# auggiemarignier/pxmcmc

Hardware: AMD Instinct MI355X
Metric: MYULA samples/sec at L=256 synthesis (higher is better)
Workload: dtype f64

## Files before the change

### pxmcmc_amd/csrc/sht_gemm.hip

```cpp
#include "../../include/pxmcmc_amd.h"
#include "sht_core.h"

#include <type_traits>

#include <hip/hip_ext.h>

#include <cstdlib>
#include <map>
#include <mutex>

namespace pxm {

typedef double d4 __attribute__((ext_vector_type(4)));

constexpr int KC = 16;
#define PXM_GEMM_MFMA(ACC, A, B) ACC = __builtin_amdgcn_mfma_f64_16x16x4f64(A, B, ACC, 0, 0, 0);
#ifdef PXM_GEMM_TRACE
__device__ unsigned long long* g_gemm_trace = nullptr;
extern "C" int pxm_debug_set_gemm_trace(unsigned long long* buf) {
  return hipMemcpyToSymbol(HIP_SYMBOL(g_gemm_trace), &buf, sizeof(buf)) == hipSuccess ? 0 : -1;
}
#endif
__device__ __forceinline__ double stage_add(double a, double b, bool on) { return a + (on ? b : 0.0); }
__device__ __forceinline__ double2 stage_add(double2 a, double2 b, bool on) { return double2{a.x + (on ? b.x : 0.0), a.y + (on ? b.y : 0.0)}; }
__device__ __forceinline__ double stage_scale(double a, double sc) { return a * sc; }
__device__ __forceinline__ double2 stage_scale(double2 a, double sc) { return double2{a.x * sc, a.y * sc}; }
template <int CT, int NSLAB>
struct GemmGeom {
  static constexpr int NCT = CT * NSLAB;
  static constexpr int COLS = 16 * NCT;
  static constexpr int PITCH = COLS + (COLS == 16 ? 0 : 16);
};
template <int CT, int NSLAB, int NW, int RT, int NSET, bool TWO, bool SK, int PK = 0, bool POLE = false>
__device__ __forceinline__ void sht_gemm_body(const GemmTask* __restrict__ tasks, const int bid,
                                              const double* __restrict__ X, double* __restrict__ Y, int ncol, int col0,
                                              const GemmAffine& aff, double (*xs)[KC][GemmGeom<CT, NSLAB>::PITCH]) {
  constexpr int NCT = CT * NSLAB;
  constexpr bool HOIST = TWO;
  constexpr int COLS = GemmGeom<CT, NSLAB>::COLS;
  constexpr int PITCH = GemmGeom<CT, NSLAB>::PITCH;
  constexpr int NT = 64 * NW;
  constexpr int VW = (KC * COLS / 2 >= NT) ? 2 : 1;
  constexpr int NV = KC * COLS / VW;
  constexpr int IT = (NV + NT - 1) / NT;
  const GemmTask t = tasks[bid];
  const int tid = threadIdx.x, lane = tid & 63;
  if (t.n_rt == 0) return;
  const int xn = (PK || TWO) ? t.x_ncol : ncol, yn = (PK || TWO) ? t.y_ncol : ncol;
#ifdef PXM_GEMM_TRACE
  const unsigned long long trace_t0 = wall_clock64();
  unsigned long long trace_t1 = 0, trace_t2 = 0;
  long long trace_c[5] = {0, 0, 0, 0, 0};
#define PXM_GEMM_CSTAMP(K) if (ch == 8) trace_c[K] = clock64();
#else
#define PXM_GEMM_CSTAMP(K)
#endif
  const int wave = __builtin_amdgcn_readfirstlane(tid >> 6);
  const int kq = lane >> 4, cl = lane & 15;
  const int n_my = min(RT, max(0, t.n_rt - RT * wave));
  const int nch = (t.k_end - t.k_beg) / KC;

  const double* sp[IT];
  const double* sp2[IT];
  const double* skp[IT];
  int so[IT];
  bool sv[IT];
#pragma unroll
  for (int i = 0; i < IT; ++i) {
    const int q0 = tid + NT * i;
    const int q = q0 % NV;
    const int kr = (q / (COLS / VW)) % KC, col = VW * (q % (COLS / VW));
    const int slab = PK ? ((col / (PK ? PK : 1)) < tasks[bid].nslab ? col / (PK ? PK : 1) : 0) : col / (16 * CT);
    const int cin = PK ? col % (PK ? PK : 1) : col % (16 * CT);
    sv[i] = q0 < NV;
    const int64_t xo = tasks[bid].x_off[slab];
    sp[i] = X + xo + col0 + cin + (int64_t)(t.k_beg + kr) * xn;
    sp2[i] = sp[i];
    skp[i] = sp[i];
    if (TWO) {
      const int64_t x2o = tasks[bid].x2_off[slab];
      if (x2o) sp2[i] = sp[i] + (x2o - xo);
    }
    if (SK) {
      const int64_t ks = tasks[bid].ks_off[slab >> 1];
      if (ks) skp[i] = X + ks + t.k_beg + kr;
    }
    so[i] = kr * PITCH + col;
  }
  const bool two = TWO && t.x2_off[0] != 0;
  const bool has_sk = SK && t.ks_off[0] != 0;
  typedef typename std::conditional<VW == 2, double2, double>::type stage_t;
  stage_t st[NSET - 1][IT], st2[NSET - 1][IT];
  double ssc[NSET - 1][IT];
#define PXM_STAGE_LOAD(SET, CH)                                                                     \
  {                                                                                                 \
    const int cs = min((CH), nch - 1);                                                              \
    _Pragma("unroll") for (int i = 0; i < IT; ++i) {                                                \
      st[SET][i] = *reinterpret_cast<const stage_t*>(sp[i] + (int64_t)cs * KC * xn);                \
      if (TWO) st2[SET][i] = *reinterpret_cast<const stage_t*>(sp2[i] + (int64_t)cs * KC * xn);   \
      if (SK) ssc[SET][i] = skp[i][cs * KC];                                                        \
    }                                                                                               \
  }
#define PXM_STAGE_STORE(SET, BUF)                                                                   \
  _Pragma("unroll") for (int i = 0; i < IT; ++i) {                                                  \
    stage_t v = st[SET][i];                                                                         \
    if (TWO) v = stage_add(v, st2[SET][i], two);                                                    \
    if (SK) {                                                                                       \
      v = stage_scale(v, has_sk ? ssc[SET][i] : 1.0);                                               \
    }                                                                                               \
    if (sv[i]) *reinterpret_cast<stage_t*>(&xs[BUF][0][0] + so[i]) = v;                             \
  }

  const double2* tab[RT];
#pragma unroll
  for (int r = 0; r < RT; ++r)
    tab[r] = reinterpret_cast<const double2*>(X + t.tab_off + (int64_t)(n_my > r ? RT * wave + r : 0) * t.rt_stride) + lane;
  const bool v0 = n_my > 0;
  double2 A[NSET][RT][2];
#define PXM_TAB_LOAD(SET, CH)                                                 \
  {                                                                           \
    const int cc = min((CH), nch - 1);                                        \
    _Pragma("unroll") for (int r = 0; r < RT; ++r) {                          \
      A[SET][r][0] = tab[r][(int64_t)(2 * cc) * 64];                          \
      A[SET][r][1] = tab[r][(int64_t)(2 * cc + 1) * 64];                      \
    }                                                                         \
  }

  d4 acc[RT][NCT];
#pragma unroll
  for (int r = 0; r < RT; ++r)
#pragma unroll
    for (int c = 0; c < NCT; ++c) acc[r][c] = d4{0, 0, 0, 0};

#pragma unroll
  for (int u = 0; u < NSET - 1; ++u)
#pragma unroll
    for (int i = 0; i < IT; ++i) {
      st[u][i] = st2[u][i] = stage_t{};
      ssc[u][i] = 0.0;
    }
  constexpr int PER = NSET * (NSET - 1);
  const int nit = nch + NSET - 1;
  for (int it0 = 0; it0 < nit; it0 += PER) {
#pragma unroll
    for (int pv = 0; pv < PER; ++pv) {
      const int it = it0 + pv;
      const int ch = it - (NSET - 1);
      constexpr int LAG = NSET - 1;
      const int us = pv % (NSET - 1);
      const int ut = pv % NSET;
      const int um = (pv + NSET - LAG % NSET) % NSET;
      const int buf = (pv + PER - LAG) & 1;
      PXM_GEMM_CSTAMP(0)
#ifdef PXM_GEMM_TRACE
      if (ch == 9) trace_c[4] = clock64();
#endif
      PXM_STAGE_STORE(us, buf)
      PXM_GEMM_CSTAMP(1)
      PXM_STAGE_LOAD(us, it)
      PXM_TAB_LOAD(ut, it)
      __syncthreads();
#ifdef PXM_GEMM_TRACE
      if (ch == 0) trace_t1 = wall_clock64();
#endif
      PXM_GEMM_CSTAMP(2)
      if (v0 && ch >= 0 && ch < nch) {
#define PXM_MFMA_CHUNK(NC)                                                                                     \
  {                                                                                                            \
    double b[4][NC];     \
    _Pragma("unroll") for (int h4 = 0; h4 < 4; ++h4)                                                           \
      _Pragma("unroll") for (int c = 0; c < NC; ++c) b[h4][c] = xs[buf][4 * h4 + kq][16 * c + cl];             \
    if (HOIST) __builtin_amdgcn_sched_barrier(0);  \
    _Pragma("unroll") for (int h4 = 0; h4 < 4; ++h4)                                                           \
      _Pragma("unroll") for (int r = 0; r < RT; ++r) {                                                         \
        const double av = (h4 & 1) ? A[um][r][h4 >> 1].y : A[um][r][h4 >> 1].x;                                \
        _Pragma("unroll") for (int c = 0; c < NC; ++c)                                                         \
            PXM_GEMM_MFMA(acc[r][c], av, b[h4][c])                                                             \
      }                                                                                                        \
  }
        PXM_MFMA_CHUNK(NCT)
#undef PXM_MFMA_CHUNK
      }
      PXM_GEMM_CSTAMP(3)
    }
  }
#undef PXM_STAGE_LOAD
#undef PXM_STAGE_STORE
#undef PXM_TAB_LOAD
#ifdef PXM_GEMM_TRACE
  trace_t2 = wall_clock64();
#endif

  constexpr int NGRP = PK ? 2 : 1;
  double hdv[RT][NSLAB][4], rsv[RT][NGRP][4];
#pragma unroll
  for (int r = 0; r < RT; ++r) {
    const int rowb = t.row0 + 16 * (r < n_my ? RT * wave + r : 0) + kq;
#pragma unroll
    for (int sl = 0; sl < NSLAB; ++sl)
#pragma unroll
      for (int q = 0; q < 4; ++q)
        hdv[r][sl][q] = (aff.on && t.hd_off[sl]) ? (X + t.hd_off[sl])[(int64_t)(rowb + 4 * q) * t.hd_stride + (cl & 1)] : 0.0;
#pragma unroll
    for (int g = 0; g < NGRP; ++g)
#pragma unroll
      for (int q = 0; q < 4; ++q) rsv[r][g][q] = t.rs_off[g] ? (X + t.rs_off[g])[rowb + 4 * q] : 1.0;
  }
  if constexpr (POLE) {
    if (t.pole_n) {
      constexpr int W2 = 8 * CT;
      constexpr int NRG = NT / W2;
      const int cp = tid % W2, rg = tid / W2;
      const double* xo = X + t.x_off[0] + t.pole_dx + col0 + 2 * cp;
      const double* xo2 = two ? X + t.x2_off[0] + t.pole_dx + col0 + 2 * cp : xo;
      const double* bo = X + t.pole_bo_off;
      double bown[RT][4];
#pragma unroll
      for (int r = 0; r < RT; ++r)
#pragma unroll
        for (int q = 0; q < 4; ++q)
          bown[r][q] = (X + t.pole_b_off)[t.row0 + 16 * (r < n_my ? RT * wave + r : 0) + kq + 4 * q];
      double2 part{0.0, 0.0};
#pragma unroll 1
      for (int r = rg; r < t.pole_n; r += NRG) {
        const double2 a = *reinterpret_cast<const double2*>(xo + (int64_t)r * xn);
        const double2 a2 = *reinterpret_cast<const double2*>(xo2 + (int64_t)r * xn);
        const double bv = bo[r];
        const double2 v = stage_add(a, a2, two);
        part.x += bv * v.x;
        part.y += bv * v.y;
      }
#pragma unroll
      for (int msk = W2; msk < 64; msk <<= 1) {
        part.x += __shfl_xor(part.x, msk);
        part.y += __shfl_xor(part.y, msk);
      }
      double* red = &xs[0][0][0];
      __syncthreads();
      if (lane < W2) *reinterpret_cast<double2*>(red + wave * 2 * W2 + 2 * lane) = part;
      __syncthreads();
#pragma unroll
      for (int ct = 0; ct < CT; ++ct) {
        double sc = 0.0;
#pragma unroll
        for (int w = 0; w < NW; ++w) sc += red[w * 2 * W2 + 16 * ct + cl];
#pragma unroll
        for (int r = 0; r < RT; ++r)
#pragma unroll
          for (int sl = 0; sl < NSLAB; ++sl)
#pragma unroll
            for (int q = 0; q < 4; ++q) acc[r][sl * CT + ct][q] += 0.5 * bown[r][q] * sc;
      }
    }
  }
  if constexpr (PK != 0) {
    const int slab = cl / PK, grp = slab >> 1;
    const bool live = slab < t.nslab;
    const double sgn = (slab & 1) ? t.sign1 : 1.0;
    const int64_t yo = tasks[bid].y_off[live ? slab : 0];
    const int row_lo = grp ? t.row_lo[1] : t.row_lo[0], row_hi = grp ? t.row_hi[1] : t.row_hi[0];
#pragma unroll
    for (int r = 0; r < RT; ++r) {
      if (r >= n_my) continue;
      const int rowb = t.row0 + 16 * (RT * wave + r) + kq;
      double* yb = Y + yo + col0 + (cl % PK) + (int64_t)rowb * yn;
#pragma unroll
      for (int q = 0; q < 4; ++q) {
        const int row = rowb + 4 * q;
        const double rs = grp ? rsv[r][NGRP - 1][q] : rsv[r][0][q];
        if (live && row >= row_lo && row < row_hi) yb[(int64_t)(4 * q) * yn] = sgn * rs * acc[r][0][q];
      }
    }
  } else {
#pragma unroll
  for (int r = 0; r < RT; ++r) {
    if (r >= n_my) continue;
#pragma unroll
    for (int c = 0; c < NCT; ++c) {
      const int slab = c / CT, cin = 16 * (c % CT), grp = slab >> 1;
      const double sgn = (slab & 1) ? t.sign1 : 1.0;
      const int rowb = t.row0 + 16 * (RT * wave + r) + kq;
      double* yb = Y + t.y_off[slab] + col0 + cin + cl + (int64_t)rowb * yn;
#pragma unroll
      for (int q = 0; q < 4; ++q) {
        const int row = rowb + 4 * q;
        double v = acc[r][c][q];
        if (aff.on) {
          const double u = aff.ns * v - hdv[r][slab][q];
          int lo = __double2loint(u), hi = __double2hiint(u);
          lo = __builtin_amdgcn_mov_dpp(lo, 0xB1, 0xF, 0xF, true);
          hi = __builtin_amdgcn_mov_dpp(hi, 0xB1, 0xF, 0xF, true);
          const double pu = __hiloint2double(hi, lo);
          v = (cl & 1) ? (aff.wr * u + aff.wi * pu) : (aff.wr * u - aff.wi * pu);
          if (col0 + cin + cl >= aff.ncol_live) v = 0.0;
        }
        if (row >= t.row_lo[grp] && row < t.row_hi[grp]) yb[(int64_t)(4 * q) * yn] = sgn * rsv[r][grp][q] * v;
      }
    }
  }
  }
#ifdef PXM_GEMM_TRACE
  __syncthreads();
  if (tid == 0 && g_gemm_trace) {
    unsigned hw, xcc;
    asm volatile("s_getreg_b32 %0, hwreg(HW_REG_HW_ID)" : "=s"(hw));
    asm volatile("s_getreg_b32 %0, hwreg(HW_REG_XCC_ID)" : "=s"(xcc));
    const unsigned long long slot = atomicAdd(g_gemm_trace, 1ull);
    unsigned long long* r = g_gemm_trace + 8 + 8 * slot;
    r[0] = blockIdx.x; r[1] = gridDim.x; r[2] = trace_t0; r[3] = wall_clock64();
    r[4] = ((unsigned long long)(xcc & 0xf) << 32) | hw; r[5] = (unsigned long long)nch | ((unsigned long long)t.n_rt << 16) | ((unsigned long long)aff.on << 32);
    r[6] = trace_t1; r[7] = trace_t2;
    if (nch > 9) {
      const unsigned long long s2 = atomicAdd(g_gemm_trace + 1, 1ull);
      unsigned long long* q = g_gemm_trace + 8 + 8 * 8192 + 8 * s2;
      q[0] = nch; q[1] = trace_c[1] - trace_c[0]; q[2] = trace_c[2] - trace_c[1]; q[3] = trace_c[3] - trace_c[2];
      q[4] = trace_c[4] - trace_c[3]; q[5] = aff.on; q[6] = gridDim.x; q[7] = 0;
    }
  }
#endif
}

template <int CT, int NSLAB, int NW, int RT, int NSET, bool TWO, bool SK, bool POLE = false>
__global__ __launch_bounds__(64 * NW) void k_sht_gemm(const GemmTask* __restrict__ tasks,
                                                      const double* __restrict__ X, double* __restrict__ Y,
                                                      int ncol, int col0, GemmAffine aff) {
  __shared__ double xs[2][KC][GemmGeom<CT, NSLAB>::PITCH];
  static_assert(!POLE || 2 * KC * GemmGeom<CT, NSLAB>::PITCH >= NW * 16 * CT, "the pole reduction borrows the operand buffers");
  if (aff.bump && blockIdx.x == 0 && threadIdx.x == 0) *aff.bump += 1;
  sht_gemm_body<CT, NSLAB, NW, RT, NSET, TWO, SK, 0, POLE>(tasks, blockIdx.x, X, Y, ncol, col0, aff, xs);
}
template <int PK, int NW, int RT, int NSET, bool TWO, bool SK>
__global__ __launch_bounds__(64 * NW) void k_sht_gemm_pk(const GemmTask* __restrict__ tasks, const double* __restrict__ X,
                                                         double* __restrict__ Y, int ncol, int col0, GemmAffine aff) {
  __shared__ double xs[2][KC][GemmGeom<1, 1>::PITCH];
  sht_gemm_body<1, 1, NW, RT, NSET, TWO, SK, PK>(tasks, blockIdx.x, X, Y, ncol, col0, aff, xs);
}

int profiler_enable(Profiler* pr, int max_launches) {
  profiler_release(pr);
  if (max_launches <= 0) return 0;
  for (Profiler::Pool* p : {&pr->gemm, &pr->dft}) {
    p->ev.resize((size_t)max_launches);
    for (auto& e : p->ev) {
      e.first = e.second = nullptr;
      PXM_HIP(hipEventCreate(&e.first));
      PXM_HIP(hipEventCreate(&e.second));
    }
  }
  pr->on = true;
  return 0;
}
void profiler_release(Profiler* pr) {
  pr->on = false;
  for (Profiler::Pool* p : {&pr->gemm, &pr->dft}) {
    for (auto& e : p->ev) {
      deferred_event_destroy(e.first);
      deferred_event_destroy(e.second);
    }
    p->ev.clear();
    p->used = 0;
    p->bytes = p->flops = 0;
    p->launch_bytes.clear();
    p->launch_wgs.clear();
  }
}
int profiler_read(Profiler::Pool* p, double* ms, int64_t* launches, double* bytes, double* flops, double* per_launch_ms,
                  double* per_launch_bytes, int64_t cap, int32_t* per_launch_wgs) {
  double tot = 0;
  for (size_t i = 0; i < p->used; ++i) {
    PXM_HIP(hipEventSynchronize(p->ev[i].second));
    float t = 0;
    PXM_HIP(hipEventElapsedTime(&t, p->ev[i].first, p->ev[i].second));
    tot += t;
    if ((int64_t)i < cap) {
      if (per_launch_ms) per_launch_ms[i] = t;
      if (per_launch_bytes) per_launch_bytes[i] = p->launch_bytes[i];
      if (per_launch_wgs) per_launch_wgs[i] = p->launch_wgs[i];
    }
  }
  if (ms) *ms = tot;
  if (launches) *launches = (int64_t)p->used;
  if (bytes) *bytes = p->bytes;
  if (flops) *flops = p->flops;
  p->used = 0;
  p->bytes = p->flops = 0;
  p->launch_bytes.clear();
  p->launch_wgs.clear();
  return 0;
}

int check_gemm_task_ranges(const std::vector<GemmTask>& v, int nslab, int flags, int ncol, const double* ws_base,
                           const char* list_name) {
  int64_t n = 0;
  std::string why;
  auto bad = [&](size_t ti, const char* what, int col0) {
    set_error(std::string("GEMM task address range outside its buffer: list '") + list_name + "', task " + std::to_string(ti) +
              ", column group " + std::to_string(col0) + ", " + what + ": " + why);
    return -1;
  };
  auto ok = [&](int64_t lo, int64_t hi) {
    ++n;
    return lo <= hi && dev_range_ok(ws_base + lo, ws_base + hi + 1, &why);
  };
  const bool TWO = flags & 1, SK = flags & 2;
  for (size_t ti = 0; ti < v.size(); ++ti) {
    const GemmTask& t = v[ti];
    if (t.n_rt == 0) continue;
    const int nch = (t.k_end - t.k_beg) / KC;
    if (!ok(t.tab_off, t.tab_off + (int64_t)(t.n_rt - 1) * t.rt_stride + (int64_t)(2 * (nch - 1) + 1) * 128 + 127))
      return bad(ti, "ring-table stream", 0);
    for (int col0 = 0; col0 < ncol && t.pole_n; col0 += 32) {
      const int CT = (ncol - col0 >= 32) ? 2 : 1;
      if (!ok(t.pole_b_off + t.row0, t.pole_b_off + t.row0 + 16 * t.n_rt - 1)) return bad(ti, "pole column of the task's rows", col0);
      if (!ok(t.pole_bo_off, t.pole_bo_off + t.pole_n - 1)) return bad(ti, "pole column of the other parity", col0);
      const int64_t lo = t.pole_dx + col0, hi = t.pole_dx + col0 + 16 * CT - 1 + (int64_t)(t.pole_n - 1) * t.x_ncol;
      if (!ok(t.x_off[0] + lo, t.x_off[0] + hi)) return bad(ti, "pole term operand", col0);
      if (t.x2_off[0] && !ok(t.x2_off[0] + lo, t.x2_off[0] + hi)) return bad(ti, "pole term second operand", col0);
    }
    for (int col0 = 0; col0 < ncol; col0 += 32) {
      const int CT = (ncol - col0 >= 32) ? 2 : 1;
      for (int slab = 0; slab < nslab; ++slab) {
        const int xn = ((TWO || nslab == 4) && t.x_ncol) ? t.x_ncol : ncol, yn = ((TWO || nslab == 4) && t.y_ncol) ? t.y_ncol : ncol;
        const int wx = std::min(16 * CT, xn), wy = std::min(16 * CT, yn);
        const int64_t lo = col0 + (int64_t)t.k_beg * xn, hi = col0 + wx - 1 + (int64_t)(t.k_end - 1) * xn;
        if (!ok(t.x_off[slab] + lo, t.x_off[slab] + hi)) return bad(ti, "operand staging", col0);
        if (TWO && t.x2_off[slab] && !ok(t.x2_off[slab] + lo, t.x2_off[slab] + hi)) return bad(ti, "second operand staging", col0);
        if (SK && t.ks_off[slab >> 1] && !ok(t.ks_off[slab >> 1] + t.k_beg, t.ks_off[slab >> 1] + t.k_end - 1))
          return bad(ti, "operand scale vector", col0);
        const int64_t r_lo = t.row0, r_hi = t.row0 + 16 * t.n_rt - 1;
        if (t.hd_off[slab] && !ok(t.hd_off[slab] + r_lo * t.hd_stride, t.hd_off[slab] + r_hi * t.hd_stride + 1))
          return bad(ti, "affine data term", col0);
        if (t.rs_off[slab >> 1] && !ok(t.rs_off[slab >> 1] + r_lo, t.rs_off[slab >> 1] + r_hi))
          return bad(ti, "per-row output scale", col0);
        const int64_t s_lo = std::max<int64_t>(r_lo, t.row_lo[slab >> 1]), s_hi = std::min<int64_t>(r_hi, (int64_t)t.row_hi[slab >> 1] - 1);
        if (s_lo <= s_hi && !ok(t.y_off[slab] + col0 + s_lo * yn, t.y_off[slab] + col0 + wy - 1 + s_hi * yn))
          return bad(ti, "result rows", col0);
      }
    }
  }
  ranges_checked_add(n);
  return 0;
}

int gemm_rows_per_task(int ncol) {
  (void)ncol;
  return 8;
}

int launch_gemm(const GemmTask* d_tasks, int n_tasks, int nslab, int flags, const double* X, double* Y, int ncol,
                int col0, int ct, double alg_bytes, double flops, hipStream_t stream, const GemmAffine& aff, Profiler* prof) {
  if (n_tasks == 0) return 0;
  PXM_REQUIRE(nslab == 1 || nslab == 2, "launch_gemm: nslab must be 1 (unpaired tables) or 2 (+-m pairs)");
  dim3 grid(n_tasks), block(512);
  hipEvent_t ev0 = nullptr, ev1 = nullptr;
  if (prof) prof->next(prof->gemm, &ev0, &ev1, alg_bytes, flops, n_tasks);
#define PXM_GEMM_L4(CT_, NS_, TWO_, SK_) \
  hipExtLaunchKernelGGL((k_sht_gemm<CT_, NS_, 8, 1, 2, TWO_, SK_>), grid, block, 0, stream, ev0, ev1, 0, d_tasks, X, Y, ncol, col0, aff)
#define PXM_GEMM_L3(CT_, NS_)                                   \
  switch (flags & 3) {                                          \
    case 0: PXM_GEMM_L4(CT_, NS_, false, false); break;         \
    case 1: PXM_GEMM_L4(CT_, NS_, true, false); break;          \
    case 2: PXM_GEMM_L4(CT_, NS_, false, true); break;          \
    default: PXM_GEMM_L4(CT_, NS_, true, true); break;          \
  }
  if (flags & 4) {
    PXM_REQUIRE(nslab == 2 && (flags & 3) == 1, "launch_gemm: a pole term outside the Gram list");
    if (ct == 1) hipExtLaunchKernelGGL((k_sht_gemm<1, 2, 8, 1, 2, true, false, true>), grid, block, 0, stream, ev0, ev1, 0, d_tasks, X, Y, ncol, col0, aff);
    else hipExtLaunchKernelGGL((k_sht_gemm<2, 2, 8, 1, 2, true, false, true>), grid, block, 0, stream, ev0, ev1, 0, d_tasks, X, Y, ncol, col0, aff);
  } else if (nslab == 2) {
    if (ct == 1) { PXM_GEMM_L3(1, 2) } else { PXM_GEMM_L3(2, 2) }
  } else {
    if (ct == 1) { PXM_GEMM_L3(1, 1) } else { PXM_GEMM_L3(2, 1) }
  }
#undef PXM_GEMM_L3
#undef PXM_GEMM_L4
  PXM_HIP(hipGetLastError());
  return 0;
}

int launch_gemm_packed(const GemmTask* d_tasks, int n_tasks, int pk, int flags, const double* X, double* Y, int ncol, int col0,
                       double alg_bytes, double flops, hipStream_t stream, Profiler* prof) {
  if (n_tasks == 0) return 0;
  PXM_REQUIRE(pk == 2 || pk == 4, "launch_gemm_packed: 2 or 4 live columns per slab");
  dim3 grid(n_tasks), block(512);
  hipEvent_t ev0 = nullptr, ev1 = nullptr;
  if (prof) prof->next(prof->gemm, &ev0, &ev1, alg_bytes, flops, n_tasks);
  GemmAffine aff;
#define PXM_PK_L(PK_, TWO_, SK_) \
  hipExtLaunchKernelGGL((k_sht_gemm_pk<PK_, 8, 1, 3, TWO_, SK_>), grid, block, 0, stream, ev0, ev1, 0, d_tasks, X, Y, ncol, col0, aff)
#define PXM_PK_N(PK_)                                     \
  switch (flags & 3) {                                    \
    case 0: PXM_PK_L(PK_, false, false); break;           \
    case 1: PXM_PK_L(PK_, true, false); break;            \
    case 2: PXM_PK_L(PK_, false, true); break;            \
    default: PXM_PK_L(PK_, true, true); break;            \
  }
  if (pk == 2) { PXM_PK_N(2) } else { PXM_PK_N(4) }
#undef PXM_PK_N
#undef PXM_PK_L
  PXM_HIP(hipGetLastError());
  return 0;
}

static void fill_side(GemmTask& g, int grp, const ShtTables& T, int kind, int m, int ncol, const GemmSide& sd,
                      int64_t scratch_off, const double* ws_base) {
  const int s0 = 2 * grp, s1 = 2 * grp + 1;
  const int xn = sd.x_ncol ? sd.x_ncol : ncol, yn = sd.y_ncol ? sd.y_ncol : ncol;
  g.x_off[s0] = sd.x_base + (int64_t)(m + sd.x_L - 1) * sd.x_Rp * xn;
  g.y_off[s0] = sd.y_base + (int64_t)(m + sd.y_L - 1) * sd.y_Rp * yn;
  if (T.paired) {
    if (m == 0) {
      g.x_off[s1] = g.x_off[s0];
      g.y_off[s1] = scratch_off;
    } else {
      g.x_off[s1] = sd.x_base + (int64_t)(-m + sd.x_L - 1) * sd.x_Rp * xn;
      g.y_off[s1] = sd.y_base + (int64_t)(-m + sd.y_L - 1) * sd.y_Rp * yn;
    }
  } else {
    g.x_off[s1] = g.x_off[s0];
    g.y_off[s1] = g.y_off[s0];
  }
  g.ks_off[grp] = sd.kscale ? (sd.kscale - ws_base) : 0;
  g.rs_off[grp] = sd.fuse.rscale ? (sd.fuse.rscale - ws_base) : 0;
  g.row_lo[grp] = sd.fuse.row_lo;
  g.row_hi[grp] = sd.fuse.row_hi;
  g.x2_off[s0] = g.x2_off[s1] = 0;
  if (sd.fuse.x2_base >= 0) {
    g.x2_off[s0] = sd.fuse.x2_base + (int64_t)(m + sd.x_L - 1) * sd.x_Rp * xn;
    g.x2_off[s1] = (T.paired && m != 0) ? sd.fuse.x2_base + (int64_t)(-m + sd.x_L - 1) * sd.x_Rp * xn : g.x2_off[s0];
  }
  g.hd_off[s0] = g.hd_off[s1] = 0;
  g.hd_stride = sd.fuse.hd_stride > 0 ? sd.fuse.hd_stride : ncol;
  if (sd.fuse.hd_base >= 0) {
    g.hd_off[s0] = sd.fuse.hd_base + (int64_t)(m + sd.y_L - 1) * sd.y_Rp * g.hd_stride;
    g.hd_off[s1] = (T.paired && m != 0) ? sd.fuse.hd_base + (int64_t)(-m + sd.y_L - 1) * sd.y_Rp * g.hd_stride : g.hd_off[s0];
  }
  (void)kind;
}

static void append_block_tasks(const ShtTables& T, int kind, int ncol, const GemmSide& side, int64_t scratch_off,
                               const double* ws_base, std::vector<GemmTask>& tasks, int m, const double* tab, int kb, int n,
                               int par, int64_t rt_stride_stored = 0, const double* pole = nullptr) {
  const bool rows_el = kind_rows_are_el(kind), k_el = kind_k_is_el(kind);
  const int lo16 = round_down(std::max(side.el_lo, 0), 16);
  const int rpt = gemm_rows_per_task(ncol);
  const int start = std::max(kb, lo16);
  if (start >= n) return;
  const int64_t rt_stride = rt_stride_stored ? rt_stride_stored : (int64_t)((k_el ? n - kb : n) / 8) * 128;
  const int k_beg = k_el ? start : 0, k_end = n, row_beg = rows_el ? start : 0;
  const int64_t tab_skip = (rows_el ? (int64_t)((start - kb) / 16) * rt_stride : 0) + (k_el ? (int64_t)((start - kb) / 8) * 128 : 0);
  const int n_rt_total = (n - row_beg) / 16;
  for (int rt = 0; rt < n_rt_total; rt += rpt) {
    GemmTask g;
    g.m_unit = T.paired ? m : m + T.L - 1;
    g.tab_off = (tab + tab_skip + (int64_t)rt * rt_stride) - ws_base;
    g.rt_stride = rt_stride;
    for (int s = 0; s < 2; ++s) fill_side(g, s, T, kind, m, ncol, side, scratch_off, ws_base);
    g.nslab = T.paired ? 2 : 1;
    g.k_beg = k_beg;
    g.k_end = k_end;
    g.row0 = row_beg + 16 * rt;
    g.n_rt = std::min(rpt, n_rt_total - rt);
    g.sign1 = kind_is_gram(kind) ? 1.0 : ((m & 1) ? -1.0 : 1.0);
    g.x_ncol = side.x_ncol ? side.x_ncol : ncol;
    g.y_ncol = side.y_ncol ? side.y_ncol : ncol;
    g.pole_n = g.pole_dx = 0;
    g.pole_b_off = g.pole_bo_off = 0;
    if (pole) {
      g.pole_n = n;
      g.pole_dx = par ? -g.x_ncol : g.x_ncol;
      g.pole_b_off = (pole + par * n) - ws_base;
      g.pole_bo_off = (pole + (1 - par) * n) - ws_base;
    }
    if (par >= 0) {
      for (int s = 0; s < 4; ++s) {
        g.x_off[s] += par * g.x_ncol;
        g.y_off[s] += par * g.y_ncol;
        if (g.x2_off[s]) g.x2_off[s] += par * g.x_ncol;
        if (g.hd_off[s]) g.hd_off[s] += par * g.hd_stride;
      }
      g.x_ncol *= 2;
      g.y_ncol *= 2;
      g.hd_stride *= 2;
      for (int grp = 0; grp < 2; ++grp) g.row_lo[grp] = round_down(m, 16) / 2;
    }
    tasks.push_back(g);
  }
}

static void append_tasks_impl(const ShtTables& T, int kind, int ncol, const GemmSide& side,
                              int64_t scratch_off, const double* ws_base, std::vector<GemmTask>& tasks) {
  for (int i = 0; i < T.n_m; ++i) {
    const int m = T.m_of(i);
    const double* tab = T.d_tab[kind] + T.m_off[kind][i];
    const int kb = T.k_beg[kind][i];
    if (kind == TAB_GRAM_SPLIT0 && m == 0) {
      const int Rh = T.Rp / 2;
      const int64_t rs = (int64_t)(T.Rp / 8) * 128;
      append_block_tasks(T, kind, ncol, side, scratch_off, ws_base, tasks, m, tab, 0, Rh, 0, rs, T.d_pole);
      append_block_tasks(T, kind, ncol, side, scratch_off, ws_base, tasks, m, tab + (Rh / 16) * rs + (int64_t)(Rh / 8) * 128, 0, Rh, 1, rs, T.d_pole);
    } else if (kind_is_gram_split(kind) && T.odd_off[i] >= 0) {
      append_block_tasks(T, kind, ncol, side, scratch_off, ws_base, tasks, m, tab, kb, T.Rp / 2, 0);
      append_block_tasks(T, kind, ncol, side, scratch_off, ws_base, tasks, m, T.d_tab[kind] + T.odd_off[i], T.odd_k_beg[i], T.Rp / 2, 1);
    } else {
      append_block_tasks(T, kind, ncol, side, scratch_off, ws_base, tasks, m, tab, kb, T.Rp, -1);
    }
  }
}

void append_gemm_tasks_packed(const ShtTables& T, int kind, int ncol, const GemmSide& side_a, const GemmSide* side_b,
                              int64_t scratch_off, const double* ws_base, std::vector<GemmTask>& tasks) {
  GemmSide sa = side_a;
  if (side_b) sa.el_lo = std::min(side_a.el_lo, side_b->el_lo);
  const size_t first = tasks.size();
  append_tasks_impl(T, kind, ncol, sa, scratch_off, ws_base, tasks);
  for (size_t i = first; i < tasks.size(); ++i) {
    GemmTask& g = tasks[i];
    const int m = T.paired ? g.m_unit : g.m_unit - (T.L - 1);
    fill_side(g, 0, T, kind, m, ncol, side_a, scratch_off, ws_base);
    fill_side(g, 1, T, kind, m, ncol, side_b ? *side_b : side_a, scratch_off, ws_base);
    g.nslab = side_b ? 4 : 2;
    g.x_ncol = side_a.x_ncol ? side_a.x_ncol : ncol;
    g.y_ncol = side_a.y_ncol ? side_a.y_ncol : ncol;
    if (!T.paired) {
      g.nslab = 1;
    }
  }
}

void append_gemm_tasks(const ShtTables& T, int kind, int ncol, int64_t x_base, int x_L, int x_Rp,
                       int64_t y_base, int y_L, int y_Rp, const double* kscale, int64_t scratch_off,
                       const double* ws_base, std::vector<GemmTask>& tasks, int el_lo, const GemmFuse& fuse) {
  const GemmSide sd{x_base, y_base, x_L, x_Rp, y_L, y_Rp, kscale, el_lo, fuse};
  append_tasks_impl(T, kind, ncol, sd, scratch_off, ws_base, tasks);
}

__global__ void k_build_fwd(const double* __restrict__ Bd, const double* __restrict__ Qd, double* __restrict__ Ad,
                            int Rp, int L, double scale, int m0, int spin) {
  const int i = blockIdx.z;
  const int el = blockIdx.x * 16 + threadIdx.x, t = blockIdx.y * 16 + threadIdx.y;
  const int m = m0 + i;
  const int par = ((m + spin) & 1) ? 1 : 0;
  const double* B = Bd + (int64_t)i * Rp * Rp;
  const double* Q = Qd + (int64_t)par * Rp * Rp;
  double acc = 0;
  for (int tp = 0; tp < L; ++tp) acc += B[(int64_t)tp * Rp + el] * Q[(int64_t)tp * Rp + t];
  Ad[(int64_t)i * Rp * Rp + (int64_t)el * Rp + t] = scale * acc;
}

__global__ void k_build_gram(const double* __restrict__ Bd, double* __restrict__ Gd, int Rp, int L) {
  const int i = blockIdx.z;
  const int r = blockIdx.x * 16 + threadIdx.x, c = blockIdx.y * 16 + threadIdx.y;
  const double* B = Bd + (int64_t)i * Rp * Rp;
  double acc = 0;
  for (int t = 0; t < L; ++t) acc += B[(int64_t)t * Rp + r] * B[(int64_t)t * Rp + c];
  Gd[(int64_t)i * Rp * Rp + (int64_t)r * Rp + c] = acc;
}

__global__ void k_tile_table(const double* __restrict__ D, double* __restrict__ out, int Rp, int n, int row_beg,
                             int k_beg, int transposed, int par) {
  const int nk2 = (n - k_beg) / 8;
  const int rt = blockIdx.y;
  const int kk2 = blockIdx.x;
  const int lane = threadIdx.x >> 1, h = threadIdx.x & 1;
  int row = row_beg + 16 * rt + (lane & 15);
  int k = k_beg + 8 * kk2 + 4 * h + (lane >> 4);
  if (par == 2) {
    row = row < n / 2 ? 2 * row : 2 * (row - n / 2) + 1;
    k = k < n / 2 ? 2 * k : 2 * (k - n / 2) + 1;
  } else if (par >= 0) {
    row = 2 * row + par;
    k = 2 * k + par;
  }
  const double v = transposed ? D[(int64_t)k * Rp + row] : D[(int64_t)row * Rp + k];
  out[((int64_t)rt * nk2 + kk2) * 128 + threadIdx.x] = v;
}

static std::mutex g_tab_mutex;
static std::map<std::pair<int, int>, ShtTables*> g_tab_cache;

static int build_gram_split(ShtTables& T, int kind, const double* d_G) {
  const int Rp = T.Rp, Rh = Rp / 2;
  PXM_REQUIRE(gram_can_split(T), "build_gram_split: the parity split needs spin-0 tables and Rp % 32 == 0");
  T.m_off[kind].assign(T.n_m, 0);
  T.k_beg[kind].assign(T.n_m, 0);
  T.odd_off.assign(T.n_m, -1);
  T.odd_k_beg.assign(T.n_m, 0);
  int64_t total = 0;
  for (int m = 0; m < T.n_m; ++m) {
    if (m == 0 || !gram_order_splits(Rp, m)) {
      const int kb = round_down(m, 16);
      T.k_beg[kind][m] = kb;
      T.m_off[kind][m] = total;
      total += (int64_t)((Rp - kb) / 16) * ((Rp - kb) / 8) * 128;
      continue;
    }
    for (int par = 0; par < 2; ++par) {
      const int kb = gram_half_k_beg(m, par);
      (par ? T.odd_k_beg[m] : T.k_beg[kind][m]) = kb;
      (par ? T.odd_off[m] : T.m_off[kind][m]) = total;
      total += (int64_t)((Rh - kb) / 16) * ((Rh - kb) / 8) * 128;
    }
  }
  T.bytes[kind] = (size_t)total * sizeof(double);
  if (int rc = dev_alloc(&T.d_tab[kind], T.bytes[kind], "ring table")) return rc;
  if (kind == TAB_GRAM_SPLIT0 && !T.d_pole) {
    if (int rc = dev_alloc(&T.d_pole, (size_t)Rp * sizeof(double), "pole column of the order-0 Gram block")) return rc;
    if (!dry_run()) {
      std::vector<double> B0((size_t)Rp * Rp, 0.0), b(Rp, 0.0);
      wigner_ring_table(T.L, 0, 0, B0.data(), Rp);
      for (int l = 0; l < T.L; ++l) b[(l & 1) * Rh + l / 2] = B0[(size_t)(T.L - 1) * Rp + l];
      if (int rc = dev_upload(T.d_pole, b.data(), b.size() * sizeof(double))) return rc;
    }
  }
  if (dry_run()) return 0;
  for (int m = 0; m < T.n_m; ++m) {
    const double* src = d_G + (int64_t)m * Rp * Rp;
    if (T.odd_off[m] < 0) {
      const int kb = T.k_beg[kind][m];
      hipLaunchKernelGGL(k_tile_table, dim3((Rp - kb) / 8, (Rp - kb) / 16), dim3(128), 0, 0, src, T.d_tab[kind] + T.m_off[kind][m],
                         Rp, Rp, kb, kb, 0, (kind == TAB_GRAM_SPLIT0 && m == 0) ? 2 : -1);
      continue;
    }
    for (int par = 0; par < 2; ++par) {
      const int kb = par ? T.odd_k_beg[m] : T.k_beg[kind][m];
      hipLaunchKernelGGL(k_tile_table, dim3((Rh - kb) / 8, (Rh - kb) / 16), dim3(128), 0, 0, src,
                         T.d_tab[kind] + (par ? T.odd_off[m] : T.m_off[kind][m]), Rp, Rh, kb, kb, 0, par);
    }
  }
  PXM_HIP(hipGetLastError());
  return 0;
}

static int build_kind(ShtTables& T, int kind, const double* d_B, const double* d_A, const double* d_G) {
  if (kind_is_gram_split(kind)) return build_gram_split(T, kind, d_G);
  const int Rp = T.Rp;
  const bool rows_el = kind_rows_are_el(kind), k_el = kind_k_is_el(kind);
  T.m_off[kind].resize(T.n_m);
  T.k_beg[kind].resize(T.n_m);
  int64_t total = 0;
  for (int i = 0; i < T.n_m; ++i) {
    const int elmin = std::max(std::abs(T.m_of(i)), std::abs(T.spin));
    const int kb = round_down(elmin, 16);
    T.k_beg[kind][i] = kb;
    T.m_off[kind][i] = total;
    total += (int64_t)((rows_el ? Rp - kb : Rp) / 16) * ((k_el ? Rp - kb : Rp) / 8) * 128;
  }
  T.bytes[kind] = (size_t)total * sizeof(double);
  if (int rc = dev_alloc(&T.d_tab[kind], T.bytes[kind], "ring table")) return rc;
  if (dry_run()) return 0;
  for (int i = 0; i < T.n_m; ++i) {
    const int kb = T.k_beg[kind][i];
    const double* src;
    int transposed;
    if (kind == TAB_INV) { src = d_B; transposed = 0; }
    else if (kind == TAB_FWD_ADJ) { src = d_A; transposed = 1; }
    else if (kind == TAB_FWD) { src = d_A; transposed = 0; }
    else if (kind == TAB_INV_ADJ) { src = d_B; transposed = 1; }
    else { src = d_G; transposed = 0; }
    src += (int64_t)i * Rp * Rp;
    const int row_beg = rows_el ? kb : 0, k_beg = k_el ? kb : 0;
    dim3 grid((Rp - k_beg) / 8, (Rp - row_beg) / 16), block(128);
    if (grid.x == 0 || grid.y == 0) continue;
    hipLaunchKernelGGL(k_tile_table, grid, block, 0, 0, src, T.d_tab[kind] + T.m_off[kind][i], Rp, Rp, row_beg, k_beg,
                       transposed, -1);
  }
  PXM_HIP(hipGetLastError());
  return 0;
}

int get_tables(int L, int spin, unsigned kinds_mask, ShtTables** out) {
  std::lock_guard<std::mutex> lock(g_tab_mutex);
  int dev = 15;
  if (!dry_run()) {
    PXM_HIP(hipGetDevice(&dev));
    PXM_REQUIRE(dev >= 0 && dev < 15, "get_tables: device index outside [0, 15)");
  }
  auto key = std::make_pair(L * 16 + dev, spin);
  ShtTables* T = nullptr;
  auto it = g_tab_cache.find(key);
  if (it != g_tab_cache.end()) T = it->second;
  else {
    T = new ShtTables();
    T->L = L;
    T->spin = spin;
    T->Rp = round_up(L, 16);
    T->paired = (spin == 0);
    T->n_m = T->paired ? L : 2 * L - 1;
    g_tab_cache[key] = T;
  }
  unsigned missing = 0;
  for (int k = 0; k < TAB_KINDS; ++k)
    if ((kinds_mask >> k & 1u) && !T->d_tab[k]) missing |= 1u << k;
  if (missing && dry_run()) {
    for (int k = 0; k < TAB_KINDS; ++k)
      if (missing >> k & 1u) {
        int rc = build_kind(*T, k, nullptr, nullptr, nullptr);
        if (rc) return rc;
      }
  } else if (missing) {
    const int Rp = T->Rp;
    const size_t dense = (size_t)T->n_m * Rp * Rp;
    std::vector<double> hB(dense, 0.0);
    const int m0 = T->paired ? 0 : -(L - 1);
    for (int i = 0; i < T->n_m; ++i) wigner_ring_table(L, spin, m0 + i, hB.data() + (size_t)i * Rp * Rp, Rp);
    double *d_B = nullptr, *d_A = nullptr, *d_Q = nullptr, *d_G = nullptr;
    PXM_HIP(hipMalloc(&d_B, dense * sizeof(double)));
    PXM_HIP(hipMemcpy(d_B, hB.data(), dense * sizeof(double), hipMemcpyHostToDevice));
    hB.clear();
    hB.shrink_to_fit();
    if (missing & ((1u << TAB_FWD) | (1u << TAB_FWD_ADJ))) {
      std::vector<double> hQ((size_t)2 * Rp * Rp, 0.0);
      quadrature_gram(L, +1, hQ.data(), Rp);
      quadrature_gram(L, -1, hQ.data() + (size_t)Rp * Rp, Rp);
      PXM_HIP(hipMalloc(&d_Q, hQ.size() * sizeof(double)));
      PXM_HIP(hipMemcpy(d_Q, hQ.data(), hQ.size() * sizeof(double), hipMemcpyHostToDevice));
      PXM_HIP(hipMalloc(&d_A, dense * sizeof(double)));
      dim3 grid(Rp / 16, Rp / 16, T->n_m), block(16, 16);
      hipLaunchKernelGGL(k_build_fwd, grid, block, 0, 0, d_B, d_Q, d_A, Rp, L, 2.0 * M_PI / (2 * L - 1), m0, spin);
      PXM_HIP(hipGetLastError());
    }
    if (missing & ((1u << TAB_GRAM) | (1u << TAB_GRAM_SPLIT) | (1u << TAB_GRAM_SPLIT0))) {
      PXM_HIP(hipMalloc(&d_G, dense * sizeof(double)));
      dim3 grid(Rp / 16, Rp / 16, T->n_m), block(16, 16);
      hipLaunchKernelGGL(k_build_gram, grid, block, 0, 0, d_B, d_G, Rp, L);
      PXM_HIP(hipGetLastError());
    }
    for (int k = 0; k < TAB_KINDS; ++k)
      if (missing >> k & 1u) {
        int rc = build_kind(*T, k, d_B, d_A, d_G);
        if (rc) return rc;
      }
    PXM_HIP(hipDeviceSynchronize());
    PXM_HIP(hipFree(d_B));
    if (d_A) PXM_HIP(hipFree(d_A));
    if (d_Q) PXM_HIP(hipFree(d_Q));
    if (d_G) PXM_HIP(hipFree(d_G));
  }
  *out = T;
  return 0;
}

void retain_tables(ShtTables* T) {
  std::lock_guard<std::mutex> lock(g_tab_mutex);
  if (T) ++T->refs;
}
void release_tables(ShtTables* T) {
  std::lock_guard<std::mutex> lock(g_tab_mutex);
  if (T && T->refs > 0) --T->refs;
}
int64_t tables_trim() {
  std::lock_guard<std::mutex> lock(g_tab_mutex);
  int64_t freed = 0;
  for (auto it = g_tab_cache.begin(); it != g_tab_cache.end();) {
    ShtTables* T = it->second;
    if (T->refs > 0 || (dry_run() && it->first.first % 16 != 15)) {
      ++it;
      continue;
    }
    for (int k = 0; k < TAB_KINDS; ++k) {
      if (T->d_tab[k]) deferred_free(T->d_tab[k]);
      freed += (int64_t)T->bytes[k];
    }
    if (T->d_pole) deferred_free(T->d_pole);
    delete T;
    it = g_tab_cache.erase(it);
  }
  drain_deferred();
  return freed;
}

}
```

Baseline: 122,300.

## Prefetch GEMM epilogue operands and pole reduction before the main loop

The epilogue's row-scale, affine-offset and pole-weight loads, along with the pole partial-sum accumulation, now run before the MFMA k-loop. Their results are parked in a new shared-memory buffer during the first pipeline iteration and read back from LDS in the epilogue. This is meant to hide the global-memory latency of those scattered loads behind the main GEMM instead of exposing it at the tail. The cost is extra LDS per block and more live registers across the loop, which could lower occupancy.

Result: faster. 126,500, median of 6 (+3.4%).

```diff
diff --git a/pxmcmc_amd/csrc/sht_gemm.hip b/pxmcmc_amd/csrc/sht_gemm.hip
--- a/pxmcmc_amd/csrc/sht_gemm.hip
+++ b/pxmcmc_amd/csrc/sht_gemm.hip
@@ -31,11 +31,21 @@
   static constexpr int COLS = 16 * NCT;
   static constexpr int PITCH = COLS + (COLS == 16 ? 0 : 16);
 };
+template <int NSLAB, int NW, int RT, bool POLE>
+struct GemmEpi {
+  static constexpr int ROWS = 16 * NW * RT;
+  static constexpr int NHD = 2 * NSLAB * ROWS;
+  static constexpr int RS_AT = NHD, B_AT = NHD + ROWS;
+  static constexpr int SIZE = NHD + ROWS + (POLE ? ROWS : 0);
+};
 template <int CT, int NSLAB, int NW, int RT, int NSET, bool TWO, bool SK, int PK = 0, bool POLE = false>
 __device__ __forceinline__ void sht_gemm_body(const GemmTask* __restrict__ tasks, const int bid,
                                               const double* __restrict__ X, double* __restrict__ Y, int ncol, int col0,
-                                              const GemmAffine& aff, double (*xs)[KC][GemmGeom<CT, NSLAB>::PITCH]) {
+                                              const GemmAffine& aff, double (*xs)[KC][GemmGeom<CT, NSLAB>::PITCH],
+                                              double* __restrict__ es) {
   constexpr int NCT = CT * NSLAB;
+  typedef GemmEpi<NSLAB, NW, RT, POLE> Epi;
+  constexpr bool EARLY = PK == 0;
   constexpr bool HOIST = TWO;
   constexpr int COLS = GemmGeom<CT, NSLAB>::COLS;
   constexpr int PITCH = GemmGeom<CT, NSLAB>::PITCH;
@@ -126,6 +136,44 @@
     }                                                                         \
   }
 
+  constexpr int EIT = (Epi::NHD + NT - 1) / NT;
+  double e_hd[EIT], e_rs = 1.0;
+  if constexpr (EARLY) {
+#pragma unroll
+    for (int i = 0; i < EIT; ++i) {
+      const int e = (tid + NT * i) % Epi::NHD, sl = e / (2 * Epi::ROWS), rl = (e >> 1) % Epi::ROWS;
+      int64_t ho = t.hd_off[0];
+#pragma unroll
+      for (int s2 = 1; s2 < NSLAB; ++s2) ho = sl == s2 ? t.hd_off[s2] : ho;
+      e_hd[i] = 0.0;
+      if (aff.on && ho) e_hd[i] = (X + ho)[(int64_t)(t.row0 + (rl < 16 * t.n_rt ? rl : 0)) * t.hd_stride + (e & 1)];
+    }
+    if (t.rs_off[0] && tid < Epi::ROWS) e_rs = (X + t.rs_off[0])[t.row0 + (tid < 16 * t.n_rt ? tid : 0)];
+  }
+  double2 part{0.0, 0.0};
+  if constexpr (POLE) {
+    if (t.pole_n) {
+      constexpr int W2 = 8 * CT;
+      constexpr int NRG = NT / W2;
+      const int cp = tid % W2, rg = tid / W2;
+      const double* xo = X + t.x_off[0] + t.pole_dx + col0 + 2 * cp;
+      const double* xo2 = two ? X + t.x2_off[0] + t.pole_dx + col0 + 2 * cp : xo;
+      const double* bo = X + t.pole_bo_off;
+      double b_own = 0.0;
+      if (tid < Epi::ROWS) b_own = (X + t.pole_b_off)[t.row0 + (tid < 16 * t.n_rt ? tid : 0)];
+#pragma unroll 1
+      for (int r = rg; r < t.pole_n; r += NRG) {
+        const double2 a = *reinterpret_cast<const double2*>(xo + (int64_t)r * xn);
+        const double2 a2 = *reinterpret_cast<const double2*>(xo2 + (int64_t)r * xn);
+        const double bv = bo[r];
+        const double2 v = stage_add(a, a2, two);
+        part.x += bv * v.x;
+        part.y += bv * v.y;
+      }
+      if (tid < Epi::ROWS) es[Epi::B_AT + tid] = b_own;
+    }
+  }
+
   d4 acc[RT][NCT];
 #pragma unroll
   for (int r = 0; r < RT; ++r)
@@ -157,6 +205,12 @@
 #endif
       PXM_STAGE_STORE(us, buf)
       PXM_GEMM_CSTAMP(1)
+      if (EARLY && pv == 1 && it0 == 0) {
+#pragma unroll
+        for (int i = 0; i < EIT; ++i)
+          if (tid + NT * i < Epi::NHD) es[tid + NT * i] = e_hd[i];
+        if (tid < Epi::ROWS) es[Epi::RS_AT + tid] = e_rs;
+      }
       PXM_STAGE_LOAD(us, it)
       PXM_TAB_LOAD(ut, it)
       __syncthreads();
@@ -195,41 +249,30 @@
   double hdv[RT][NSLAB][4], rsv[RT][NGRP][4];
 #pragma unroll
   for (int r = 0; r < RT; ++r) {
-    const int rowb = t.row0 + 16 * (r < n_my ? RT * wave + r : 0) + kq;
-#pragma unroll
-    for (int sl = 0; sl < NSLAB; ++sl)
-#pragma unroll
-      for (int q = 0; q < 4; ++q)
-        hdv[r][sl][q] = (aff.on && t.hd_off[sl]) ? (X + t.hd_off[sl])[(int64_t)(rowb + 4 * q) * t.hd_stride + (cl & 1)] : 0.0;
-#pragma unroll
-    for (int g = 0; g < NGRP; ++g)
-#pragma unroll
-      for (int q = 0; q < 4; ++q) rsv[r][g][q] = t.rs_off[g] ? (X + t.rs_off[g])[rowb + 4 * q] : 1.0;
+    const int rl = 16 * (r < n_my ? RT * wave + r : 0) + kq;
+    const int rowb = t.row0 + rl;
+    if constexpr (EARLY) {
+#pragma unroll
+      for (int sl = 0; sl < NSLAB; ++sl)
+#pragma unroll
+        for (int q = 0; q < 4; ++q) hdv[r][sl][q] = es[2 * (sl * Epi::ROWS + rl + 4 * q) + (cl & 1)];
+#pragma unroll
+      for (int q = 0; q < 4; ++q) rsv[r][0][q] = es[Epi::RS_AT + rl + 4 * q];
+    } else {
+#pragma unroll
+      for (int g = 0; g < NGRP; ++g)
+#pragma unroll
+        for (int q = 0; q < 4; ++q) rsv[r][g][q] = t.rs_off[g] ? (X + t.rs_off[g])[rowb + 4 * q] : 1.0;
+    }
   }
   if constexpr (POLE) {
     if (t.pole_n) {
       constexpr int W2 = 8 * CT;
-      constexpr int NRG = NT / W2;
-      const int cp = tid % W2, rg = tid / W2;
-      const double* xo = X + t.x_off[0] + t.pole_dx + col0 + 2 * cp;
-      const double* xo2 = two ? X + t.x2_off[0] + t.pole_dx + col0 + 2 * cp : xo;
-      const double* bo = X + t.pole_bo_off;
       double bown[RT][4];
 #pragma unroll
       for (int r = 0; r < RT; ++r)
 #pragma unroll
-        for (int q = 0; q < 4; ++q)
-          bown[r][q] = (X + t.pole_b_off)[t.row0 + 16 * (r < n_my ? RT * wave + r : 0) + kq + 4 * q];
-      double2 part{0.0, 0.0};
-#pragma unroll 1
-      for (int r = rg; r < t.pole_n; r += NRG) {
-        const double2 a = *reinterpret_cast<const double2*>(xo + (int64_t)r * xn);
-        const double2 a2 = *reinterpret_cast<const double2*>(xo2 + (int64_t)r * xn);
-        const double bv = bo[r];
-        const double2 v = stage_add(a, a2, two);
-        part.x += bv * v.x;
-        part.y += bv * v.y;
-      }
+        for (int q = 0; q < 4; ++q) bown[r][q] = es[Epi::B_AT + 16 * (r < n_my ? RT * wave + r : 0) + kq + 4 * q];
 #pragma unroll
       for (int msk = W2; msk < 64; msk <<= 1) {
         part.x += __shfl_xor(part.x, msk);
@@ -325,15 +368,16 @@
                                                       const double* __restrict__ X, double* __restrict__ Y,
                                                       int ncol, int col0, GemmAffine aff) {
   __shared__ double xs[2][KC][GemmGeom<CT, NSLAB>::PITCH];
+  __shared__ double es[GemmEpi<NSLAB, NW, RT, POLE>::SIZE];
   static_assert(!POLE || 2 * KC * GemmGeom<CT, NSLAB>::PITCH >= NW * 16 * CT, "the pole reduction borrows the operand buffers");
   if (aff.bump && blockIdx.x == 0 && threadIdx.x == 0) *aff.bump += 1;
-  sht_gemm_body<CT, NSLAB, NW, RT, NSET, TWO, SK, 0, POLE>(tasks, blockIdx.x, X, Y, ncol, col0, aff, xs);
+  sht_gemm_body<CT, NSLAB, NW, RT, NSET, TWO, SK, 0, POLE>(tasks, blockIdx.x, X, Y, ncol, col0, aff, xs, es);
 }
 template <int PK, int NW, int RT, int NSET, bool TWO, bool SK>
 __global__ __launch_bounds__(64 * NW) void k_sht_gemm_pk(const GemmTask* __restrict__ tasks, const double* __restrict__ X,
                                                          double* __restrict__ Y, int ncol, int col0, GemmAffine aff) {
   __shared__ double xs[2][KC][GemmGeom<1, 1>::PITCH];
-  sht_gemm_body<1, 1, NW, RT, NSET, TWO, SK, PK>(tasks, blockIdx.x, X, Y, ncol, col0, aff, xs);
+  sht_gemm_body<1, 1, NW, RT, NSET, TWO, SK, PK>(tasks, blockIdx.x, X, Y, ncol, col0, aff, xs, nullptr);
 }
 
 int profiler_enable(Profiler* pr, int max_launches) {
```
